# alibaba/unified-audio

Hardware: AMD Instinct MI355X
Metric: audio-seconds/sec H-Codec encode+decode @16kHz b=32 (higher is better)
Workload: dtype f32

## Files before the change

unified_audio_amd/csrc/conv_gemm.hip:

```cpp
#include <algorithm>
#include <cstdlib>
#include <type_traits>

#include "common.h"
#include "split_planes.h"

#ifndef QA_LOAD_AT
#define QA_LOAD_AT 0
#endif

#ifdef QA_TIMING
__device__ unsigned long long g_qa_timing[10];
extern "C" int qa_debug_timing(unsigned long long* out, int reset) {
    if (out && hipMemcpyFromSymbol(out, HIP_SYMBOL(g_qa_timing), sizeof(g_qa_timing)) != hipSuccess) return -1;
    if (reset) {
        unsigned long long z[10] = {0};
        if (hipMemcpyToSymbol(HIP_SYMBOL(g_qa_timing), z, sizeof(z)) != hipSuccess) return -1;
    }
    return 0;
}
#endif

namespace qa {

// ... 392 lines not shown
                    p.am_idx[m * p.am_ld + (ep_n >> 5)] = bi;
                }
                continue;
            }
            if (m >= p.M || ep_n >= p.N) continue;
            f32x4 v = *reinterpret_cast<const f32x4*>(stage + r * EP_LD + 4 * ep_c4);
            if (p.vec_epi) {
                v = epilogue4(v, p, m, ep_n, bias4, gamma4);
                *reinterpret_cast<f32x4*>(p.y + m * p.ldy + ep_n) = v;
            } else {
                for (int e = 0; e < 4 && ep_n + e < p.N; ++e) {
                    const int n = ep_n + e;
                    float u = v[e] + (p.bias ? p.bias[n] : 0.f);
                    if (p.gate) u = silu_f(p.gate[m * p.ldg + n]) * u;
                    u = apply_act(u, p.act);
                    if (p.gamma) u *= p.gamma[n];
                    if (p.res) u += p.res[m * p.ldr + n];
                    u = apply_act(u, p.post_act);
                    p.y[m * p.ldy + n] = u;
                }
            }
        }
    });
#ifdef QA_TIMING
    if (lane == 0) {
        const long long tend = __builtin_readcyclecounter();
        atomicAdd(&g_qa_timing[4], (unsigned long long)(tend - tloop));
        atomicAdd(&g_qa_timing[5], (unsigned long long)(tend - tbegin));
        atomicAdd(&g_qa_timing[6], 1ULL);
        atomicAdd(&g_qa_timing[7], (unsigned long long)nk);
        atomicAdd(&g_qa_timing[8], __builtin_amdgcn_s_memrealtime() - rbegin);
    }
#endif
}

static bool is_linear(const ConvParams& p) {
    return knob(K_GEMM_LINEAR) != 0 && p.ksize == 1 && p.stride == 1 && p.pad_left == 0 && p.in_rep <= 1 && p.T_in == p.T_out && p.dilation <= 1;
}

constexpr int prof_cfg(int bm, int bn) {
    return bm == 256 ? PROF_CFG_256x128 : bm == 64 ? (bn == 64 ? PROF_CFG_64x64 : PROF_CFG_64x128) : bn == 32 ? PROF_CFG_128x32 : bn == 64 ? PROF_CFG_128x64 : PROF_CFG_128x128;
}

template <int BM, int BN, int WM, int WN, bool ELU, int BK, bool LIN>
static void launch_instance(const ConvParams& p, long long tiles, hipStream_t stream) {
    const bool split = knob(K_GEMM_MATH) != 0 && !p.math_fp32;
    constexpr bool IMAGE = BN == 128;
    const auto kernel = !split            ? conv_gemm_kernel<BM, BN, WM, WN, ELU, BK, LIN, false, false>
                        : IMAGE && p.wp ? conv_gemm_kernel<BM, BN, WM, WN, ELU, BK, LIN, true, IMAGE>
                                        : conv_gemm_kernel<BM, BN, WM, WN, ELU, BK, LIN, true, false>;
    hipLaunchKernelGGL(kernel, dim3((unsigned)tiles), dim3(256), 0, stream, p);
}

template <int BM, int BN, int WM, int WN>
static int launch_cfg(const ConvParams& p, hipStream_t stream) {
    QA_REQUIRE(p.prologue == ACT_NONE || p.prologue == ACT_ELU, "conv_gemm: prologue %d unsupported", p.prologue);
    const long long tiles = ceil_div(p.M, BM) * ceil_div(p.N, BN);
    const long long bk16_max_k = knob(K_GEMM_BK16);
    const long long bk16_min_tiles = knob(K_GEMM_BK16_MIN_TILES);
    const bool linear = is_linear(p), elu = p.prologue == ACT_ELU;
    const bool bk16 = BM == 256 || (BN >= 64 && !elu && ((p.K <= bk16_max_k && tiles >= bk16_min_tiles) || p.C_in % 32 != 0));
    const int bk = bk16 ? 16 : 32;
    const bool table = BM != 256 && (!linear || elu);
    QA_REQUIRE(p.K % bk == 0 && (!table || p.C_in % bk == 0),
               "conv_gemm: the %dx%d tile's BK = %d K chunk does not divide K=%d / C_in=%d", BM, BN, bk, p.K, p.C_in);
    const bool prof = profile_enabled();
    if (prof) {
        const double n = p.algo_n ? p.algo_n : p.N, k = p.algo_k ? p.algo_k : p.K;
        const double out_elems = p.am_dist ? 2.0 * (double)p.M * p.am_ld + p.M + n
                                            : (double)p.M * n * (1.0 + (p.res ? 1.0 : 0.0) + (p.gate ? 1.0 : 0.0));
        const double elems = (double)p.B * p.T_in * p.C_in + n * k + out_elems;
        profile_record_begin(prof_cfg(BM, BN), 2.0 * (double)p.M * n * k, 4.0 * elems, stream, &p);
    }
    if constexpr (BM == 256) QA_REQUIRE(linear && !elu, "conv_gemm: the 256 x 128 tile exists for LINEAR layers only");
    constexpr int BK16 = BN >= 64 ? 16 : 32;
    if (bk16 && linear) launch_instance<BM, BN, WM, WN, false, BK16, true>(p, tiles, stream);
    else if constexpr (BM != 256) {
        if (bk16) launch_instance<BM, BN, WM, WN, false, BK16, false>(p, tiles, stream);
        else if (elu) launch_instance<BM, BN, WM, WN, true, 32, false>(p, tiles, stream);
        else if (linear) launch_instance<BM, BN, WM, WN, false, 32, true>(p, tiles, stream);
        else launch_instance<BM, BN, WM, WN, false, 32, false>(p, tiles, stream);
    }
    if (prof) profile_record_end(stream);
    QA_LAUNCH_CHECK();
    return QA_OK;
}

static int choose_tile(const ConvParams& p) {
    const bool lin = is_linear(p) && p.prologue != ACT_ELU;
    int cfg = (int)knob(K_GEMM_CFG);
    if (cfg < 0) {
        if (p.N <= 32) cfg = PROF_CFG_128x32;
        else if (p.N <= 64) cfg = PROF_CFG_128x64;
        else {
            struct Cand { int cfg, bm, bn; double eff; };
            static const Cand cands[] = {{PROF_CFG_128x128, 128, 128, 1.0}, {PROF_CFG_64x128, 64, 128, 0.914}, {PROF_CFG_128x64, 128, 64, 0.913},
                                         {PROF_CFG_64x64, 64, 64, 0.871}};
            auto cost_of = [&](int bm, int bn, double eff) {
                const long long tiles = ceil_div(p.M, bm) * ceil_div(p.N, bn);
                return (double)ceil_div(tiles, 256) * bm * bn / eff * (tiles <= 256 ? 1.25 : 1.0);
            };
            double best = 0.0;
            cfg = PROF_CFG_128x128;
            const long long eff256 = knob(K_GEMM_256);
            if (eff256 > 0 && lin && p.M >= 8000 && p.N >= 1024) {
                best = cost_of(256, 128, eff256 / 1000.0);
                cfg = PROF_CFG_256x128;
            }
            for (const Cand& c : cands) {
                const double cost = cost_of(c.bm, c.bn, c.eff);
                if (best == 0.0 || cost < best * 0.995) {
                    best = cost;
                    cfg = c.cfg;
                }
            }
        }
    }
    if (cfg == PROF_CFG_128x32 && p.C_in % 32 != 0) return PROF_CFG_128x64;
    if ((cfg == PROF_CFG_256x128 && !lin) || cfg >= PROF_NCFG) return PROF_CFG_128x128;
    return cfg;
}

int launch_conv_gemm(const ConvParams& p, hipStream_t stream) {
    QA_REQUIRE(p.K % 16 == 0 && p.C_in % 16 == 0, "conv_gemm: K=%d / C_in=%d must be multiples of 16", p.K, p.C_in);
    QA_REQUIRE(p.C_in % 32 == 0 || (p.N > 32 && p.prologue != ACT_ELU),
               "conv_gemm: C_in=%d is not a multiple of 32 (only supported for N > 32 without the ELU prologue)", p.C_in);
    QA_REQUIRE((p.ldx % 4) == 0, "conv_gemm: ldx=%lld must be a multiple of 4 floats", p.ldx);
    QA_REQUIRE((long long)p.T_in * p.ldx < (1LL << 31), "conv_gemm: one batch item spans %lld floats (limit 2^31)",
               (long long)p.T_in * p.ldx);
    QA_REQUIRE(((uintptr_t)p.x % 16) == 0 && ((uintptr_t)p.w % 16) == 0, "conv_gemm: x / w must be 16-byte aligned");
    if (p.M <= 0 || p.N <= 0) return QA_OK;
    QA_REQUIRE(ceil_div(p.M, 64) * ceil_div(p.N, 32) < (1LL << 31), "conv_gemm: grid too large");
    auto al16 = [](const void* ptr) { return ((uintptr_t)ptr % 16) == 0; };
    const bool vec_epi = p.N % 4 == 0 && p.ldy % 4 == 0 && al16(p.y) && (!p.bias || al16(p.bias)) && (!p.gamma || al16(p.gamma)) &&
                         (!p.res || (p.ldr % 4 == 0 && al16(p.res))) && (!p.gate || (p.ldg % 4 == 0 && al16(p.gate)));
    QA_REQUIRE(p.in_rep <= 1 || p.pad_mode == PAD_ZERO, "conv_gemm: in_rep needs zero padding");
    const bool snake = p.act == ACT_SNAKE || p.post_act == ACT_SNAKE;
    QA_REQUIRE((!snake && !p.y2) || (vec_epi && (!snake || (p.alpha && al16(p.alpha))) &&
                                     (!p.y2 || (p.alpha2 && al16(p.alpha2) && al16(p.y2) && p.ldy2 % 4 == 0))),
               "conv_gemm: Snake activation / second output need the float4 epilogue and 16-byte aligned alpha vectors");
    QA_REQUIRE(p.dilation <= 1 || (p.pad_mode == PAD_ZERO && p.in_rep <= 1), "conv_gemm: dilation needs zero padding");
    QA_REQUIRE(!p.am_dist || (vec_epi && p.am_idx && p.am_x2 && p.am_e2 && al16(p.am_e2) && p.am_ld >= (p.N + 31) / 32 && !p.y2),
               "conv_gemm: the arg-min epilogue needs N %% 4 == 0, x2 / e2 / dist / idx and am_ld >= ceil(N / 32)");
    QA_REQUIRE(!p.rope || (vec_epi && p.rope_hd % 4 == 0 && p.rope_n % 4 == 0 && p.rope_T > 0 && al16(p.rope)),
               "conv_gemm: fused RoPE needs the float4 epilogue (N, strides, pointers multiples of 4 / 16 B)");
    ConvParams q = p;
    q.xcd_swizzle = (int)knob(K_GEMM_XCD);
    q.panel = (int)knob(K_GEMM_PANEL);
    q.wp = knob(K_GEMM_PRESPLIT) != 0 ? weight_planes_find(p.w, (long long)p.N * p.K) : nullptr;
    q.vec_epi = vec_epi;
    q.rep_one = p.in_rep > 1 ? 0u : 1u;
    q.rep_magic = p.in_rep > 1 ? (unsigned)(((1ULL << 32) + p.in_rep - 1) / p.in_rep) : 0u;

    switch (choose_tile(p)) {
        case PROF_CFG_128x32: return launch_cfg<128, 32, 4, 1>(q, stream);
        case PROF_CFG_128x64: return launch_cfg<128, 64, 2, 2>(q, stream);
        case PROF_CFG_64x128: return launch_cfg<64, 128, 1, 4>(q, stream);
        case PROF_CFG_64x64: return launch_cfg<64, 64, 2, 2>(q, stream);
        case PROF_CFG_256x128: return launch_cfg<256, 128, 2, 2>(q, stream);
        default: return launch_cfg<128, 128, 2, 2>(q, stream);
    }
}

int conv_params_from_args(const qa_conv_args& a, ConvParams* out) {
    ConvParams p{};
    QA_REQUIRE(a.x && a.w && a.y, "conv1d_cl: x, w, y must be non-null");
    QA_REQUIRE(a.B > 0 && a.T_in > 0 && a.C_in > 0 && a.N > 0 && a.T_out >= 0, "conv1d_cl: bad shape");
    QA_REQUIRE(a.ksize >= 1 && a.stride >= 1 && a.pad_left >= 0 && a.pad_right >= 0, "conv1d_cl: bad geometry");
    QA_REQUIRE(a.B * a.T_out < (1LL << 31) && a.ksize * a.C_in < (1LL << 31), "conv1d_cl: shape too large");
    p.x = a.x; p.w = a.w; p.bias = a.bias; p.gamma = a.gamma; p.res = a.residual; p.gate = a.gate; p.y = a.y;
    p.ldx = a.ldx ? a.ldx : a.C_in;
    p.ldy = a.ldy ? a.ldy : a.N;
    p.ldr = a.ldr ? a.ldr : a.N;
    p.ldg = a.ldg ? a.ldg : a.N;
    p.B = (int)a.B; p.T_in = (int)a.T_in; p.C_in = (int)a.C_in; p.T_out = (int)a.T_out; p.N = (int)a.N;
    p.K = (int)(a.ksize * a.C_in);
    p.M = (int)(a.B * a.T_out);
    p.ksize = a.ksize; p.stride = a.stride; p.pad_left = a.pad_left; p.pad_mode = a.pad_mode;
    const int max_pad = a.pad_left > a.pad_right ? a.pad_left : a.pad_right;
    p.Lp = (p.T_in <= max_pad) ? max_pad + 1 : p.T_in;
    p.in_rep = a.in_rep > 1 ? a.in_rep : 1;
    QA_REQUIRE(a.T_out == 0 || (a.T_out - 1) * (int64_t)a.stride + a.ksize <= a.pad_left + a.T_in * (int64_t)p.in_rep + a.pad_right,
               "conv1d_cl: T_out=%lld windows do not fit pad_left=%d + T_in=%lld + pad_right=%d", (long long)a.T_out,
               a.pad_left, (long long)a.T_in, a.pad_right);
    p.prologue = a.prologue; p.act = a.act; p.post_act = a.post_act;
    *out = p;
    return QA_OK;
}

}
```

unified_audio_amd/csrc/ew.hip:

```cpp
#include "kernels.h"

namespace qa {

__global__ __launch_bounds__(256) void conv_in_kernel(const float* __restrict__ x, const float* __restrict__ w,
                                                      const float* __restrict__ bias, float* __restrict__ y, int B,
                                                      int T, int Cout, int ksize, int pad_left, int Lp) {
    const int c4n = Cout >> 2;
    const long long gid = (long long)blockIdx.x * blockDim.x + threadIdx.x;
    const long long total = (long long)B * T * c4n;
    if (gid >= total) return;
    const int c4 = (int)(gid % c4n);
    const long long m = gid / c4n;
    const int b = (int)(m / T), t = (int)(m - (long long)b * T);
    const float* xb = x + (long long)b * T;
    float4 acc = bias ? *reinterpret_cast<const float4*>(bias + c4 * 4) : make_float4(0.f, 0.f, 0.f, 0.f);
    for (int j = 0; j < ksize; ++j) {
        const int src = resolve_frame(t - pad_left + j, T, Lp, PAD_REFLECT);
        const float xv = src >= 0 ? xb[src] : 0.f;
        const float* wj = w + (long long)j * Cout + c4 * 4;
        acc.x = fmaf(xv, wj[0], acc.x);
        acc.y = fmaf(xv, wj[1], acc.y);
        acc.z = fmaf(xv, wj[2], acc.z);
        acc.w = fmaf(xv, wj[3], acc.w);
    }
// ... 510 lines not shown
    if (p < T) {
        const int dst = p + seg[(long long)b * T + p];
        for (int c = threadIdx.x * 4; c < D; c += blockDim.x * 4)
            *reinterpret_cast<float4*>(ob + (long long)dst * D + c) =
                *reinterpret_cast<const float4*>(feats + ((long long)b * T + p) * D + c);
        return;
    }
    const int g = p - T;
    if (g >= nseg[b]) {
        for (int c = threadIdx.x * 4; c < D; c += blockDim.x * 4)
            *reinterpret_cast<float4*>(ob + (long long)(T + g) * D + c) = *reinterpret_cast<const float4*>(qemb + c);
        return;
    }
    const int st = start[(long long)b * T + g], n = len[(long long)b * T + g];
    const int dst = st + n + g;
    const float inv = 1.f / (float)n;
    for (int c = threadIdx.x * 4; c < D; c += blockDim.x * 4) {
        float4 acc = make_float4(0.f, 0.f, 0.f, 0.f);
        for (int t = st; t < st + n; ++t) {
            const float4 v = *reinterpret_cast<const float4*>(feats + ((long long)b * T + t) * D + c);
            acc.x += v.x; acc.y += v.y; acc.z += v.z; acc.w += v.w;
        }
        const float4 q = *reinterpret_cast<const float4*>(qemb + c);
        acc.x = acc.x * inv + q.x; acc.y = acc.y * inv + q.y; acc.z = acc.z * inv + q.z; acc.w = acc.w * inv + q.w;
        *reinterpret_cast<float4*>(ob + (long long)dst * D + c) = acc;
    }
}
int launch_agg_build(const float* feats, const int* seg, const int* start, const int* len, const int* nseg, const float* qemb,
                     float* out, int B, int T, int G, int D, hipStream_t s) {
    hipLaunchKernelGGL(agg_build_kernel, dim3(T + G, B), dim3(128), 0, s, feats, seg, start, len, nseg, qemb, out, T, G, D);
    QA_LAUNCH_CHECK();
    return QA_OK;
}

__global__ __launch_bounds__(128) void agg_gather_kernel(const float* __restrict__ x, const int* __restrict__ start,
                                                         const int* __restrict__ len, const int* __restrict__ nseg,
                                                         float* __restrict__ out, int T, int G, int D) {
    const int b = blockIdx.y, g = blockIdx.x;
    const bool valid = g < nseg[b];
    const int src = valid ? start[(long long)b * T + g] + len[(long long)b * T + g] + g : 0;
    for (int c = threadIdx.x * 4; c < D; c += blockDim.x * 4) {
        float4 v = make_float4(0.f, 0.f, 0.f, 0.f);
        if (valid) v = *reinterpret_cast<const float4*>(x + ((long long)b * (T + G) + src) * D + c);
        *reinterpret_cast<float4*>(out + ((long long)b * G + g) * D + c) = v;
    }
}
int launch_agg_gather(const float* x, const int* start, const int* len, const int* nseg, float* out, int B, int T, int G,
                      int D, hipStream_t s) {
    hipLaunchKernelGGL(agg_gather_kernel, dim3(G, B), dim3(128), 0, s, x, start, len, nseg, out, T, G, D);
    QA_LAUNCH_CHECK();
    return QA_OK;
}

__global__ void codes_inject_kernel(const long long* __restrict__ idx, const int* __restrict__ len, long long* __restrict__ dst,
                                    int B, int T, int G, int Q, int K) {
    const long long gid = (long long)blockIdx.x * blockDim.x + threadIdx.x;
    if (gid >= (long long)B * Q * G) return;
    const int g = (int)(gid % G);
    const int q = (int)((gid / G) % Q);
    const int b = (int)(gid / ((long long)G * Q));
    dst[gid] = (long long)(len[(long long)b * T + g] - 1) * K + idx[((long long)b * G + g) * Q + q];
}
int launch_codes_inject(const long long* idx, const int* len, long long* dst, int B, int T, int G, int Q, int K,
                        hipStream_t s) {
    const long long total = (long long)B * Q * G;
    hipLaunchKernelGGL(codes_inject_kernel, dim3((unsigned)ceil_div(total, 256)), dim3(256), 0, s, idx, len, dst, B, T, G, Q, K);
    QA_LAUNCH_CHECK();
    return QA_OK;
}

__device__ __forceinline__ long long floordiv_ll(long long a, long long b) {
    long long q = a / b;
    if ((a % b != 0) && ((a < 0) != (b < 0))) --q;
    return q;
}

__global__ void adaptive_frames_kernel(const long long* __restrict__ codes, int B, int Q, int G, int K, int* __restrict__ totals,
                                       int* __restrict__ tmax) {
    const int b = blockIdx.x * blockDim.x + threadIdx.x;
    if (b >= B) return;
    int tot = 0;
    for (int g = 0; g < G; ++g) {
        const long long l = floordiv_ll(codes[((long long)b * Q) * G + g], K) + 1;
        tot += l > 0 ? (int)l : 0;
    }
    totals[b] = tot;
    atomicMax(tmax, tot);
}
int launch_adaptive_frames(const long long* codes, int B, int Q, int G, int K, int* totals, int* tmax, hipStream_t s) {
    QA_HIP(hipMemsetAsync(tmax, 0, sizeof(int), s));
    hipLaunchKernelGGL(adaptive_frames_kernel, dim3((unsigned)ceil_div(B, 64)), dim3(64), 0, s, codes, B, Q, G, K, totals, tmax);
    QA_LAUNCH_CHECK();
    return QA_OK;
}

__global__ void token_lengths_kernel(const long long* __restrict__ codes, long long* __restrict__ out, int B, int Q, int G, int K) {
    const long long gid = (long long)blockIdx.x * blockDim.x + threadIdx.x;
    if (gid >= (long long)B * G) return;
    const int g = (int)(gid % G), b = (int)(gid / G);
    out[gid] = floordiv_ll(codes[((long long)b * Q) * G + g], K) + 1;
}
int launch_token_lengths(const long long* codes, long long* out, int B, int Q, int G, int K, hipStream_t s) {
    const long long total = (long long)B * G;
    if (total == 0) return QA_OK;
    hipLaunchKernelGGL(token_lengths_kernel, dim3((unsigned)ceil_div(total, 256)), dim3(256), 0, s, codes, out, B, Q, G, K);
    QA_LAUNCH_CHECK();
// ... 125 lines not shown
```

unified_audio_amd/csrc/hcodec.cpp:

```cpp
#include <memory>

#include "host_util.h"

namespace qa {

namespace {

struct TransformerLayerW {
    const float *ln1, *ln2;
    ConvW ih;
    const float* w_hh;
    ConvW qkv, o, w1, w3, w2;
};

struct TransformerW {
    std::vector<TransformerLayerW> layers;
    int d = 0, heads = 0, inter = 0;
    const float* rope = nullptr;
};

struct ResBlockW {
    ConvW k3, pw, sc;
};
struct DecResW {
// ... 271 lines not shown
        QA_TRY(linear_op(c, hn, rows, L.w3, big2, epi(ACT_NONE, nullptr, nullptr, big)));
        QA_TRY(linear_op(c, big2, rows, L.w2, x, epi(ACT_NONE, x)));
        c.tap(lp + ".x_mlp", x, rows * d);
    }
    c.arena.release(mark);
    return QA_OK;
}

struct MimiTemps {
    float *hn, *qkv, *att, *u;
};
MimiTemps mimi_temps(Ctx& c, const MimiW& mw, int64_t rows) {
    MimiTemps t;
    t.hn = c.arena.alloc<float>(rows * mw.d);
    t.qkv = c.arena.alloc<float>(rows * 3 * mw.d);
    t.att = c.arena.alloc<float>(rows * mw.d);
    t.u = c.arena.alloc<float>(rows * mw.ff);
    return t;
}
int mimi_layer(Ctx& c, const MimiW& mw, const MimiLayerW& L, float* x, const MimiTemps& t, int B, int N, MimiStream* st = nullptr,
               size_t li = 0) {
    const int d = mw.d, H = mw.heads, hd = d / H;
    const int64_t rows = (int64_t)B * N;
    const int pos0 = st ? st->offset : 0;
    const bool win = st && st->rope_len > 0;
    const float* rope = win ? st->rope_win : mw.rope;
    const int rope_pos0 = win ? pos0 - st->rope_base : pos0;
    const float scale = 1.0f / std::sqrt((float)hd);
    QA_TRY(layernorm_op(c, x, L.n1w, L.n1b, t.hn, rows, d, 1e-5f));
    ConvOpt qo;
    qo.rope = rope; qo.rope_n = 2 * d; qo.rope_hd = hd; qo.rope_T = N; qo.rope_pos0 = rope_pos0;
    QA_TRY(linear_op(c, t.hn, rows, L.in_proj, t.qkv, qo));
    if (st) {
        QA_RUN(c, launch_ring_append(t.qkv + d, t.qkv + 2 * d, 3 * d, st->kc[li], st->vc[li], B, N, d, st->cap, pos0, c.stream));
        QA_TRY(attention_op(c, t.qkv, 3 * d, st->kc[li], st->vc[li], d, t.att, d, B, N, st->cap, (long long)st->cap * d, H, hd, scale, 1,
                            nullptr, nullptr, 0, mw.context, pos0, pos0 + N));
    } else {
        QA_TRY(attention_op(c, t.qkv, 3 * d, t.qkv + d, t.qkv + 2 * d, 3 * d, t.att, d, B, N, N, (long long)N * 3 * d, H, hd, scale,
                            mw.causal, nullptr, nullptr, 0, mw.causal ? mw.context : 0));
    }
    QA_TRY(linear_op(c, t.att, rows, L.out_proj, x, epi(ACT_NONE, x, L.ls1)));
    QA_TRY(layernorm_op(c, x, L.n2w, L.n2b, t.hn, rows, d, 1e-5f));
    QA_TRY(linear_op(c, t.hn, rows, L.lin1, t.u, epi(ACT_GELU)));
    return linear_op(c, t.u, rows, L.lin2, x, epi(ACT_NONE, x, L.ls2));
}
int mimi_op(Ctx& c, const MimiW& mw, float* x, int B, int N) {
    QA_REQUIRE(N <= MAX_POS, "mimi transformer: sequence of %d tokens exceeds %d", N, MAX_POS);
    const size_t mark = c.arena.mark();
    const MimiTemps t = mimi_temps(c, mw, (int64_t)B * N);
    for (const MimiLayerW& L : mw.layers) QA_TRY(mimi_layer(c, mw, L, x, t, B, N));
    c.arena.release(mark);
    return QA_OK;
}
int mimi_pair_op(Ctx& c, hipStream_t side, const MimiW& wa, float* xa, const MimiW& wb, float* xb, int B, int N) {
    QA_REQUIRE(N <= MAX_POS && wa.layers.size() == wb.layers.size(), "mimi pair: mismatched stacks");
    const size_t mark = c.arena.mark();
    const MimiTemps ta = mimi_temps(c, wa, (int64_t)B * N);
    const MimiTemps tb = mimi_temps(c, wb, (int64_t)B * N);
    if (!c.dry) {
        hipStream_t main = c.stream;
        for (size_t l = 0; l < wa.layers.size(); ++l) {
            c.stream = main;
            int st = mimi_layer(c, wa, wa.layers[l], xa, ta, B, N);
            c.stream = side;
            if (st == QA_OK) st = mimi_layer(c, wb, wb.layers[l], xb, tb, B, N);
            c.stream = main;
            QA_TRY(st);
        }
    }
    c.arena.release(mark);
    return QA_OK;
}

int groupnorm_op(Ctx& c, const float* x, const float* w, const float* b, float* y, int B, int T, int C, int G,
                 int swish) {
    const size_t mark = c.arena.mark();
    double* scratch = c.arena.alloc<double>(groupnorm_scratch_bytes(B, T, G) / sizeof(double));
    QA_RUN(c, launch_groupnorm(x, w, b, y, scratch, B, T, C, G, 1e-6f, swish, c.stream));
    c.arena.release(mark);
    return QA_OK;
}

int dec_resblock_op(Ctx& c, const DecResW& w, float* x, int B, int T, int C, int G, bool causal = false) {
    const size_t mark = c.arena.mark();
    float* t1 = c.arena.alloc<float>((size_t)B * T * C);
    float* t2 = c.arena.alloc<float>((size_t)B * T * C);
    QA_TRY(groupnorm_op(c, x, w.n1w, w.n1b, t1, B, T, C, G, 1));
    QA_TRY(conv_same(c, t1, B, T, w.c1, t2, ACT_NONE, ACT_NONE, nullptr, causal));
    QA_TRY(groupnorm_op(c, t2, w.n2w, w.n2b, t1, B, T, C, G, 1));
    QA_TRY(conv_same(c, t1, B, T, w.c2, x, ACT_NONE, ACT_NONE, x, causal));
    c.arena.release(mark);
    return QA_OK;
}


int convnext_op(Ctx& c, const ConvNeXtW& w, float* x, float* t1, float* u, int B, int T, int d, bool causal = false) {
    const int64_t rows = (int64_t)B * T;
    QA_TRY(dwconv_op(c, x, w.dw, w.dwb, w.lnw, w.lnb, t1, B, T, d, 7, 1e-6f, zpad_left(7, causal)));
    QA_TRY(linear_op(c, t1, rows, w.pw1, u, epi(ACT_GELU)));
    return linear_op(c, u, rows, w.pw2, x, epi(ACT_NONE, x, w.gamma));
}

int encoder20(qa_hcodec* h, Ctx& c, const float* wav, int B, int T, float** emb_out, int* n50_out, int* nf_out) {
    const qa_hcodec_spec& sp = h->spec;
    const int blk = (sp.n_fft - sp.hop) / 2;
    const int N50 = T / sp.hop, d = sp.enc_dim, nb = sp.n_fft / 2 + 1;
    const int64_t rows = (int64_t)B * N50;
    float* ri = c.arena.alloc<float>(rows * 2 * nb);
    QA_TRY(conv_op(c, wav, blk, B, T / blk, h->stft_basis, ri, 2 * nb, N50, conv_geom(2, 1, 1)));
    float* feat = c.arena.alloc<float>(rows * h->stft_ld);
    QA_RUN(c, launch_stft_post(ri, feat, rows, nb, 2 * nb, h->stft_ld, c.stream));
    c.tap("enc.stft", feat, rows * h->stft_ld);
    float* x = c.arena.alloc<float>(rows * d);
    float* t1 = c.arena.alloc<float>(rows * d);
    float* u = c.arena.alloc<float>(rows * sp.enc_inter);
    const bool cz = sp.causal != 0;
    QA_TRY(conv_op(c, feat, h->stft_ld, B, N50, h->enc_embed, t1, d, N50, conv_geom(1, cz ? 2 : 1, cz ? 0 : 1)));
    QA_TRY(layernorm_op(c, t1, h->enc_norm_w, h->enc_norm_b, x, rows, d, 1e-6f));
// ... 179 lines not shown
    c.tap("dec.backbone", t1, rows * d);
    const int nb = sp.n_fft / 2 + 1;
    float* y = c.arena.alloc<float>(rows * 2 * nb);
    float* S = c.arena.alloc<float>(rows * h->spec_ld);
    float* frames = c.arena.alloc<float>(rows * sp.n_fft);
    QA_TRY(linear_op(c, t1, rows, h->head, y));
    QA_RUN(c, launch_istft_spec(y, S, rows, nb, 2 * nb, h->spec_ld, c.stream));
    c.tap("dec.spec", S, rows * h->spec_ld);
    QA_TRY(linear_op(c, S, rows, h->basis, frames));
    QA_RUN(c, launch_istft_ola(frames, h->window, wav_out, B, N50, sp.n_fft, sp.hop, c.stream));
    return QA_OK;
}


int read_scalar(Ctx& c, qa_hcodec* h, const int* dev, int* out) {
    QA_HIP(hipMemcpyAsync(h->host_sync, dev, sizeof(int), hipMemcpyDeviceToHost, c.stream));
    QA_HIP(hipStreamSynchronize(c.stream));
    lstm_call_note_sync();
    *out = *h->host_sync;
    return QA_OK;
}

int encode_adaptive_graph(qa_hcodec* h, Ctx& c, const float* wav, int B, int T, const float* feat, int64_t fsb, int64_t fsc,
                          int64_t fst, int n_feat, long long* ac_out, long long* sc_out, int* G_out, float threshold) {
    const qa_hcodec_spec& sp = h->spec;
    const int D = sp.code_dim, Q = sp.num_quantizers;
    float *emb = nullptr, *sem = nullptr;
    int N = 0;
    QA_TRY(encode_front(h, c, wav, B, T, feat, fsb, fsc, fst, n_feat, &emb, &sem, &N));
    int* seg = c.arena.alloc<int>((size_t)B * N);
    int* start = c.arena.alloc<int>((size_t)B * N);
    int* len = c.arena.alloc<int>((size_t)B * N);
    int* nseg = c.arena.alloc<int>(B);
    int* gmax = c.arena.alloc<int>(1);
    int G = N;
    if (!c.dry) {
        QA_TRY(launch_align(sem, B, N, D, threshold, sp.max_tokens_per_group, seg, start, len, nseg, gmax, c.stream));
        QA_TRY(read_scalar(c, h, gmax, &G));
        QA_REQUIRE(G >= 1 && G <= N, "encode: alignment produced %d groups for %d frames", G, N);
    }
    *G_out = G;
    const int S = N + G;
    float* inter_s = c.arena.alloc<float>((size_t)B * S * D);
    float* inter_a = c.arena.alloc<float>((size_t)B * S * D);
    float* agg_a = c.arena.alloc<float>((size_t)B * G * D);
    float* agg_s = c.arena.alloc<float>((size_t)B * G * D);
    hipStream_t side = serial_mode() ? c.stream : h->side;
    QA_RUN(c, launch_agg_build(sem, seg, start, len, nseg, h->qemb_sem, inter_s, B, N, G, D, c.stream));
    QA_RUN(c, launch_agg_build(emb, seg, start, len, nseg, h->qemb_ac, inter_a, B, N, G, D, c.stream));
    if (!c.dry) {
        QA_HIP(hipEventRecord(h->ev_fork, c.stream));
        QA_HIP(hipStreamWaitEvent(side, h->ev_fork, 0));
    }
    QA_TRY(mimi_pair_op(c, side, h->agg_sem, inter_s, h->agg_ac, inter_a, B, S));
    QA_RUN(c, launch_agg_gather(inter_s, start, len, nseg, agg_s, B, N, G, D, c.stream));
    QA_RUN(c, launch_agg_gather(inter_a, start, len, nseg, agg_a, B, N, G, D, side));
    if (!c.dry) {
        QA_HIP(hipEventRecord(h->ev_join, side));
        QA_HIP(hipStreamWaitEvent(c.stream, h->ev_join, 0));
    }
    c.tap("enc.emb_agg", agg_a, (int64_t)B * G * D);
    c.tap("enc.sem_agg", agg_s, (int64_t)B * G * D);
    long long* ia = c.arena.alloc<long long>((size_t)B * G * Q);
    long long* is = c.arena.alloc<long long>((size_t)B * G * Q);
    float* rvq_ws = c.arena.alloc<float>(rvq_scratch_floats((long long)B * G, sp.codebook_size, D));
    QA_RUN(c, launch_rvq_search(agg_a, (long long)B * G, h->cb_a, h->e2_a, Q, sp.codebook_size, D, ia, nullptr, 0, rvq_ws, c.stream));
    QA_RUN(c, launch_rvq_search(agg_s, (long long)B * G, h->cb_s, h->e2_s, Q, sp.codebook_size, D, is, nullptr, 0, rvq_ws, c.stream));
    QA_RUN(c, launch_codes_inject(ia, len, ac_out, B, N, G, Q, sp.codebook_size, c.stream));
    QA_RUN(c, launch_codes_inject(is, len, sc_out, B, N, G, Q, sp.codebook_size, c.stream));
    return QA_OK;
}

int decode_adaptive_graph(qa_hcodec* h, Ctx& c, const long long* ac, const long long* scodes, int B, int G, int N,
                          float* wav_out) {
    const qa_hcodec_spec& sp = h->spec;
    const int Q = sp.num_quantizers, D = sp.code_dim;
    const int64_t rows = (int64_t)B * N;
    long long* ia = c.arena.alloc<long long>(rows * Q);
    long long* is = c.arena.alloc<long long>(rows * Q);
    float* cat = c.arena.alloc<float>(rows * 2 * D);
    QA_RUN(c, launch_deaggregate(ac, scodes, ia, B, Q, G, N, sp.codebook_size, c.stream));
    QA_RUN(c, launch_deaggregate(scodes, scodes, is, B, Q, G, N, sp.codebook_size, c.stream));
    QA_RUN(c, launch_rvq_lookup(ia, rows, h->cb_a, Q, sp.codebook_size, D, cat, 2 * D, c.stream));
    QA_RUN(c, launch_rvq_lookup(is, rows, h->cb_s, Q, sp.codebook_size, D, cat + D, 2 * D, c.stream));
    QA_TRY(mimi_op(c, h->bottleneck, cat, B, N));
    c.tap("dec.bottleneck", cat, rows * 2 * D);
    return decode_tail(h, c, cat, B, N, wav_out);
}


int semantic_decoder_op(const qa_hcodec::SemDec& sd, Ctx& c, const float* z, int64_t ldz, int B, int N, float* pred) {
    const qa_semantic_decoder_spec& sp = sd.spec;
    int L = N, C = sp.channels;
    float* x = c.arena.alloc<float>((size_t)B * L * C);
    QA_TRY(conv_op(c, z, ldz, B, L, sd.conv1, x, C, L, conv_geom(1, 1, 1)));
    for (const auto& blk : sd.blocks) {
        const int s = blk.stride, co = blk.c_out, To = L * s;
        float* y = c.arena.alloc<float>((size_t)B * To * co);
        if (s == 1) {
            QA_TRY(conv_same(c, x, B, L, blk.conv, y));
        } else {
            for (int phi = 0; phi < s; ++phi) {
                const ConvW& w = blk.phase[phi];
                QA_TRY(conv_op(c, x, C, B, L, w, y + (size_t)phi * co, (int64_t)s * co, L,
                               conv_geom(1, blk.pad_left[phi], w.ksize - 1 - blk.pad_left[phi])));
            }
        }
        float* t = c.arena.alloc<float>((size_t)B * To * co);
        for (int u = 0; u < 2; ++u) {
// ... 666 lines not shown
```

unified_audio_amd/csrc/kernels.h:

```cpp
#pragma once
#include <algorithm>

#include "common.h"

namespace qa {

int launch_conv_in(const float* x, const float* w_kc, const float* bias, float* y, int B, int T, int Cout, int ksize,
                   hipStream_t s, int pad_left = -1);
bool seanet_front_supported(int C, int hid, int L);
int launch_seanet_front(const float* wav, const float* w0, const float* b0, const float* w3, const float* b3, const float* wsc,
                        const float* bsc, const float* wpw, const float* bpw, float* a, int B, int L, int C, int hid, int causal,
                        hipStream_t s);
int launch_rmsnorm(const float* x, const float* w, float* y, long long rows, int C, float eps, hipStream_t s);
int launch_layernorm(const float* x, const float* w, const float* b, float* y, long long rows, int C, float eps,
                     hipStream_t s);
int launch_dwconv(const float* x, const float* w_kc, const float* bias, const float* lnw, const float* lnb, float* y,
                  int B, int T, int C, int ksize, float eps, hipStream_t s, int pad_left = -1);
size_t groupnorm_scratch_bytes(int B, int T, int G);
int launch_groupnorm(const float* x, const float* w, const float* bias, float* y, double* scratch, int B, int T, int C,
                     int G, float eps, int swish, hipStream_t s);
int launch_rope(float* qkv, const float* cos_sin, int B, int N, int H, int hd, long long ld, int pos0, hipStream_t s,
                int interleaved = 0, int rot_heads = 0);
int launch_align(const float* sem, int B, int T, int D, float thr, int max_tokens, int* seg, int* start, int* len,
                 int* nseg, int* gmax, hipStream_t s);
int launch_agg_build(const float* feats, const int* seg, const int* start, const int* len, const int* nseg, const float* qemb,
                     float* out, int B, int T, int G, int D, hipStream_t s);
int launch_agg_gather(const float* x, const int* start, const int* len, const int* nseg, float* out, int B, int T, int G,
                      int D, hipStream_t s);
int launch_codes_inject(const long long* idx, const int* len, long long* dst, int B, int T, int G, int Q, int K,
                        hipStream_t s);
int launch_adaptive_frames(const long long* codes, int B, int Q, int G, int K, int* totals, int* tmax, hipStream_t s);
int launch_token_lengths(const long long* codes, long long* out, int B, int Q, int G, int K, hipStream_t s);
int launch_deaggregate(const long long* codes, const long long* len_codes, long long* out, int B, int Q, int G, int T, int K,
                       hipStream_t s);
int launch_to_channel_last(const float* x, long long sb, long long sc, long long st, float* y, int B, int C, int T,
                           hipStream_t s);
int launch_codes_to_bqn(const long long* src, long long* dst, int B, int N, int Q, hipStream_t s);
int launch_codes_from_bqn(const long long* src, long long* dst, int B, int N, int Q, hipStream_t s);
int launch_stft_post(const float* ri, float* out, long long rows, int nb, int ldi, int ldo, hipStream_t s);
int launch_istft_spec(const float* y, float* S, long long rows, int nb, int ldy, int ldS, hipStream_t s);
int launch_istft_ola(const float* frames, const float* win, float* out, int B, int T, int n_fft, int hop, hipStream_t s);

int launch_codes_check(const long long* codes, long long n, long long limit, unsigned long long* bad, hipStream_t s);
int launch_codes_count(const long long* codes, long long n, long long lo, long long limit, unsigned long long* bad, hipStream_t s);
int launch_resample(const float* wav, const float* taps, float* out, int B, long long T, long long T_out, int orig, int nw, int width,
                    int ktaps, hipStream_t s);

int launch_attention(const float* q, long long ldq, const float* k, const float* v, long long ldkv, float* out,
                     long long ldo, int B, int n_q, int n_keys, long long kv_batch_stride, int H, int hd, float scale,
                     int causal, hipStream_t s, const float* gate = nullptr, const float* relbias = nullptr, int R = 0,
                     int context = 0, int q_pos0 = 0, int ring_end = 0, const unsigned char* kvalid = nullptr, bool math_fp32 = false);
int launch_ring_append(const float* k, const float* v, long long ld, float* kc, float* vc, int B, int T, int d, int cap, int pos0,
                       hipStream_t s);

int launch_lstm(const float* xw, const float* w_hh_ug, float* h_out, float* c_state, int B, int T, int d,
                hipStream_t s, bool eager = false);
int lstm_call_begin(int dev, void** ticket);
int lstm_call_end(void* ticket, hipStream_t s, bool* failed);
void lstm_call_note_sync();
void lstm_force_per_step(bool on);

size_t rvq_scratch_floats(long long n_vec, int K, int D);
int launch_rvq_search(const float* x, long long n_vec, const float* codebooks, const float* e2, int Q, int K, int D,
                      long long* indices, float* quantized, long long ldq, float* scratch, hipStream_t s);
int launch_rvq_norms(const float* codebooks, float* e2, int QK, int D, hipStream_t s);
int launch_rvq_lookup(const long long* indices, long long n_vec, const float* codebooks, int Q, int K, int D, float* out,
                      long long ldo, hipStream_t s);

int launch_assemble_prompt(float* x, const float* task_vec, const float* enroll_sos, const float* enroll_emb,
                           const float* mix_sos, const float* mix_emb, int B, int Ne, int Nm, int d, hipStream_t s,
                           const int* off = nullptr);
int launch_skinny_gemm(const float* x, long long ldx, const float* w, const float* bias, const float* gate, long long ldg,
                       const float* res, long long ldr, float* y, long long ldy, int M, int N, int K, int act, hipStream_t s,
                       float rms_eps, int dual);
int launch_rope_kv(float* qkv, const float* cs, float* kc, float* vc, int B, int n, int H, int hd, int pos0, int max_len,
                   hipStream_t s);
int launch_lm_targets(float* x, long long ldx_seq, const float* table, const long long* gids, int G, const long long* sids, int T, int V,
                      int goff, int soff, long long* tgt, int B, int d, hipStream_t s, int drop = 0);
int launch_lm_row_loss(const float* z, long long ldl, int V, long long rows, const long long* tgt, float c, float sm, float* row_kl,
                       int* row_ok, hipStream_t s);
int launch_lm_seq_reduce(const float* row_kl, const int* row_ok, int B, int Lt, double* seq_sum, float* loss_seq, long long* correct_seq,
// ... 53 lines not shown
```

unified_audio_amd/csrc/knobs.h:

```cpp
#pragma once
#include <cstdint>

namespace qa {

#define QA_KNOB_TABLE(X)                                                                                                           \
    X(SERIAL, "QA_SERIAL", 0, "1: no internal stream concurrency (every kernel alone on the device; = qa_set_serial)")           \
    X(GEMM_CFG, "QA_GEMM_CFG", -1, "force the conv_gemm tile: 0 = 128x32, 1 = 128x64, 2 = 128x128, 3 = 64x128, 4 = 64x64, 5 = 256x128 (LINEAR layers; else 128x128) (-1: cost model)")             \
    X(GEMM_256, "QA_GEMM_256", 0, "r06 experiment: 256x128 block tile (4 waves, 4x2 accumulators each) for LINEAR layers with M >= 8000 and N >= 1024; value = its efficiency relative to 128x128 in 1/1000 for the cost model (0: never chosen; QA_GEMM_CFG=5 forces it)") \
    X(GEMM_BK16, "QA_GEMM_BK16", 1 << 30, "largest K that takes the BK = 16 K-chunk variant")                                     \
    X(GEMM_BK16_MIN_TILES, "QA_GEMM_BK16_MIN_TILES", 384, "fewest tiles of a launch that take BK = 16")                          \
    X(GEMM_MATH, "QA_GEMM_MATH", 1, "conv_gemm arithmetic: 1 = split-6 (operands split into three bf16 planes, six v_mfma_f32_32x32x16_bf16 per 16-wide k group, fp32 accumulation), 0 = the fp32 chain (v_mfma_f32_32x32x2_f32)") \
    X(GEMM_PRESPLIT, "QA_GEMM_PRESPLIT", 1, "split-6 weights from a pre-split image: a weight store builds the three bf16 planes of all its weights once, at load (6 bytes per weight beside the fp32 blob; not built when 0 at load time), and conv_gemm's 128-column tiles copy them into LDS instead of splitting the weight tile in the K loop (narrower tiles keep the in-loop split); 0 at launch = ignore the image and split in the loop; same bits either way") \
    X(GEMM_LINEAR, "QA_GEMM_LINEAR", 1, "table-free K loop for ksize-1 layers")                                                  \
    X(GEMM_XCD, "QA_GEMM_XCD", 1, "XCD-aware tile order")                                                                        \
    X(GEMM_PANEL, "QA_GEMM_PANEL", 8, "conv_gemm tile order: column panels of this many tiles, row tiles fastest inside a panel (0: column tiles fastest over the whole row; 8: +4 % on N >= 4096 shapes, +1.2 % on H-Codec 2.0)") \
    X(ATT_MATH, "QA_ATT_MATH", 1, "attention arithmetic: 1 = split-6 (Q, K, V and the probabilities as three bf16 planes, six v_mfma_f32_32x32x16_bf16 per 16-wide k group, fp32 accumulation), 0 = the fp32 chain (v_mfma_f32_32x32x2_f32); the UniSE LM keeps the fp32 chain either way") \
    X(ATT_DEBUG, "QA_ATT_DEBUG", 0, "attention_kernel debug bits, both forms: 1 always rescale, 2 extra barrier per tile, 4 wait for the prefetch at once, 8 no wave-uniform tile skip, 16 mask every tile; the split-6 form (SPLIT) only (tests): 32 / 64 / 128 zero the h / m / l plane of the operands selected by 256 Q, 512 K, 1024 V, 2048 P (none of the four: all)") \
    X(SEANET_FUSED, "QA_SEANET_FUSED", 1, "fused conv0 + first SEANet residual block")                                           \
    X(MIMI_ROPE_WINDOW, "QA_MIMI_ROPE_WINDOW", 8192, "mimi streaming: positions covered by the RoPE table before the rolling window takes over (tests shrink it)") \
    X(LSTM_GRAPH, "QA_LSTM_GRAPH", 1, "replay the T step launches of an LSTM call from a cached hipGraph")                       \
    X(LSTM_PERSISTENT, "QA_LSTM_PERSISTENT", -1, "persistent recurrence kernel: -1 auto (d >= 1536), 0 off, 1 on for every supported width") \
    X(LSTM_XCD, "QA_LSTM_XCD", 1, "XCD-local LSTM recurrence for d = 512 / 768 (one launch, W_hh in the registers of every XCD's 32 CUs, sequences dealt to the XCDs, 32-member step barrier per XCD): 0 off (the per-step kernels), 1 agent-scope hand-off forms, 2 XCD-local forms (h stores that stay in the XCD's L2; H-Codec 1.0: 42.7 against 43.3 ms)") \
    X(LSTM_TEAM, "QA_LSTM_TEAM", 1, "team recurrence for d = 1024 (one launch: 4 teams of 64 workgroups, W_hh resident in registers, 8 sequences per team, agent-scope hand-offs; H-Codec 1.5 decoder: 134.1 -> 128.3 ms per step, profiles/r04_lstm_team_ab.txt): 0 = the per-step kernels") \
    X(LSTM_SPIN_LIMIT, "QA_LSTM_SPIN_LIMIT", 1 << 21, "persistent recurrence: polls of a barrier word before the barrier is declared broken") \
    X(LSTM_FAULT, "QA_LSTM_FAULT", 0, "1 (tests): the persistent kernel's barrier waits for a workgroup that does not exist, like a starved launch") \
    X(LM_GRAPH, "QA_LM_GRAPH", 0, "1: replay one captured decode step per token")                                                \
    X(LM_MLP_FUSED, "QA_LM_MLP_FUSED", 1, "decode step: gate/up + SwiGLU + down of 16 activation columns per workgroup in one launch emitting K-slice partials, summed by a reduce launch (0: separate gate/up and down launches)") \
    X(LM_PF, "QA_LM_PF", 7, "decode step: cross-launch L2 weight prefetch planes (bit mask; lm_decode.h PfArgs): 1 qkv launch -> o_proj weights, 2 o_proj launch -> fused-MLP weights, 4 MLP launch -> next layer's qkv weights (last layer: the head slice), 8 head launch -> layer 0 qkv weights") \
    X(LM_ROWSPLIT, "QA_LM_ROWSPLIT", 3, "decode step at 9 .. 16 sequences: two 8-row groups instead of one 16-row group in the qkv launch (bit 1) and the fused-MLP launch (bit 2)") \
    X(LM_CHAINS, "QA_LM_CHAINS", 0, "generate: number of concurrent chains on internal streams (0: ceil(B / 64) - one chain serves up to 64 sequences, two row groups of 32 per launch; a count that would put more than 64 sequences into a chain is raised)") \
    X(LM_SCORE_ROWS, "QA_LM_SCORE_ROWS", 4096, "qa_lm_score: target rows per output_head launch (the logits buffer holds this many rows of the full vocabulary; any value gives the same bits)")

enum Knob {
#define QA_KNOB_ENUM(id, name, def, doc) K_##id,
    QA_KNOB_TABLE(QA_KNOB_ENUM)
#undef QA_KNOB_ENUM
        K_COUNT
};

long long knob(Knob k);
void knob_set(Knob k, long long v);

}
```

Before: 3139.

## Compute only read-out rows in last aggregator layer; occupancy-aware GEMM tile cost

Result: faster. 3272, median of 6 (+4.2%).

```diff
diff --git a/unified_audio_amd/csrc/conv_gemm.hip b/unified_audio_amd/csrc/conv_gemm.hip
--- a/unified_audio_amd/csrc/conv_gemm.hip
+++ b/unified_audio_amd/csrc/conv_gemm.hip
@@ -468,14 +468,16 @@
     hipLaunchKernelGGL(kernel, dim3((unsigned)tiles), dim3(256), 0, stream, p);
 }
 
+static bool takes_bk16(int bm, int bn, long long tiles, int K, int C_in, bool elu) {
+    return bm == 256 || (bn >= 64 && !elu && ((K <= knob(K_GEMM_BK16) && tiles >= knob(K_GEMM_BK16_MIN_TILES)) || C_in % 32 != 0));
+}
+
 template <int BM, int BN, int WM, int WN>
 static int launch_cfg(const ConvParams& p, hipStream_t stream) {
     QA_REQUIRE(p.prologue == ACT_NONE || p.prologue == ACT_ELU, "conv_gemm: prologue %d unsupported", p.prologue);
     const long long tiles = ceil_div(p.M, BM) * ceil_div(p.N, BN);
-    const long long bk16_max_k = knob(K_GEMM_BK16);
-    const long long bk16_min_tiles = knob(K_GEMM_BK16_MIN_TILES);
     const bool linear = is_linear(p), elu = p.prologue == ACT_ELU;
-    const bool bk16 = BM == 256 || (BN >= 64 && !elu && ((p.K <= bk16_max_k && tiles >= bk16_min_tiles) || p.C_in % 32 != 0));
+    const bool bk16 = takes_bk16(BM, BN, tiles, p.K, p.C_in, elu);
     const int bk = bk16 ? 16 : 32;
     const bool table = BM != 256 && (!linear || elu);
     QA_REQUIRE(p.K % bk == 0 && (!table || p.C_in % bk == 0),
@@ -502,29 +504,56 @@
     return QA_OK;
 }
 
-static int choose_tile(const ConvParams& p) {
-    const bool lin = is_linear(p) && p.prologue != ACT_ELU;
+struct TileQuery {
+    long long M, N, K;
+    int C_in;
+    bool lin, elu, split;
+    bool image;
+    int share;
+};
+static int workgroups_per_cu(int cfg, bool bk16, bool split) {
+    switch (cfg) {
+        case PROF_CFG_128x128: return bk16 ? 3 : split ? 1 : 2;
+        case PROF_CFG_64x128: return bk16 ? 4 : 2;
+        case PROF_CFG_128x64: return bk16 ? 4 : 2;
+        case PROF_CFG_64x64: return bk16 ? 5 : split ? 3 : 4;
+        case PROF_CFG_256x128: return 2;
+        default: return split ? 2 : 3;
+    }
+}
+static double tile_cost(const TileQuery& t, int cfg, int bm, int bn, double eff) {
+    constexpr double kTile = 128.0 * 128.0, kRamp = 0.22, kLaunch = 0.27 * 512.0;
+    const long long tiles = ceil_div(t.M, bm) * ceil_div(t.N, bn);
+    const long long w = workgroups_per_cu(cfg, takes_bk16(bm, bn, tiles, (int)t.K, t.C_in, t.elu), t.split);
+    const long long n = tiles * (t.share > 1 ? t.share : 1), cap = 256 * w;
+    const long long rounds = ceil_div(n, cap), m = n - (rounds - 1) * cap;
+    double last = 0.5 * ((double)ceil_div(m, 256) + (double)m / 256.0);
+    if (last < 1.0) last = 1.0;
+    return kTile * kLaunch + (double)t.K * ((double)bm * bn / eff * ((double)(w * (rounds - 1)) + last) + kRamp * kTile * (double)rounds);
+}
+static double tile_cost_r4(const TileQuery& t, int bm, int bn, double eff) {
+    const long long tiles = ceil_div(t.M, bm) * ceil_div(t.N, bn);
+    return (double)ceil_div(tiles, 256) * bm * bn / eff * (tiles <= 256 ? 1.25 : 1.0);
+}
+static int choose_tile(const TileQuery& t) {
     int cfg = (int)knob(K_GEMM_CFG);
     if (cfg < 0) {
-        if (p.N <= 32) cfg = PROF_CFG_128x32;
-        else if (p.N <= 64) cfg = PROF_CFG_128x64;
+        if (t.N <= 32) cfg = PROF_CFG_128x32;
+        else if (t.N <= 64) cfg = PROF_CFG_128x64;
         else {
-            struct Cand { int cfg, bm, bn; double eff; };
-            static const Cand cands[] = {{PROF_CFG_128x128, 128, 128, 1.0}, {PROF_CFG_64x128, 64, 128, 0.914}, {PROF_CFG_128x64, 128, 64, 0.913},
-                                         {PROF_CFG_64x64, 64, 64, 0.871}};
-            auto cost_of = [&](int bm, int bn, double eff) {
-                const long long tiles = ceil_div(p.M, bm) * ceil_div(p.N, bn);
-                return (double)ceil_div(tiles, 256) * bm * bn / eff * (tiles <= 256 ? 1.25 : 1.0);
-            };
+            struct Cand { int cfg, bm, bn; double eff6, eff32; };
+            static const Cand cands[] = {{PROF_CFG_128x128, 128, 128, 1.0, 1.0}, {PROF_CFG_64x128, 64, 128, 0.85, 0.914},
+                                         {PROF_CFG_128x64, 128, 64, 0.80, 0.913}, {PROF_CFG_64x64, 64, 64, 0.69, 0.871}};
             double best = 0.0;
             cfg = PROF_CFG_128x128;
             const long long eff256 = knob(K_GEMM_256);
-            if (eff256 > 0 && lin && p.M >= 8000 && p.N >= 1024) {
-                best = cost_of(256, 128, eff256 / 1000.0);
+            const bool r4 = t.split && !t.image;
+            if (eff256 > 0 && t.lin && t.M >= 8000 && t.N >= 1024) {
+                best = r4 ? tile_cost_r4(t, 256, 128, eff256 / 1000.0) : tile_cost(t, PROF_CFG_256x128, 256, 128, eff256 / 1000.0);
                 cfg = PROF_CFG_256x128;
             }
             for (const Cand& c : cands) {
-                const double cost = cost_of(c.bm, c.bn, c.eff);
+                const double cost = r4 ? tile_cost_r4(t, c.bm, c.bn, c.eff32) : tile_cost(t, c.cfg, c.bm, c.bn, t.split ? c.eff6 : c.eff32);
                 if (best == 0.0 || cost < best * 0.995) {
                     best = cost;
                     cfg = c.cfg;
@@ -532,9 +561,13 @@
             }
         }
     }
-    if (cfg == PROF_CFG_128x32 && p.C_in % 32 != 0) return PROF_CFG_128x64;
-    if ((cfg == PROF_CFG_256x128 && !lin) || cfg >= PROF_NCFG) return PROF_CFG_128x128;
+    if (cfg == PROF_CFG_128x32 && t.C_in % 32 != 0) return PROF_CFG_128x64;
+    if ((cfg == PROF_CFG_256x128 && !t.lin) || cfg >= PROF_NCFG) return PROF_CFG_128x128;
     return cfg;
+}
+static int choose_tile(const ConvParams& p) {
+    const bool elu = p.prologue == ACT_ELU;
+    return choose_tile(TileQuery{p.M, p.N, p.K, p.C_in, is_linear(p) && !elu, elu, knob(K_GEMM_MATH) != 0 && !p.math_fp32, p.wp != nullptr, 1});
 }
 
 int launch_conv_gemm(const ConvParams& p, hipStream_t stream) {
@@ -568,7 +601,7 @@
     q.rep_one = p.in_rep > 1 ? 0u : 1u;
     q.rep_magic = p.in_rep > 1 ? (unsigned)(((1ULL << 32) + p.in_rep - 1) / p.in_rep) : 0u;
 
-    switch (choose_tile(p)) {
+    switch (choose_tile(q)) {
         case PROF_CFG_128x32: return launch_cfg<128, 32, 4, 1>(q, stream);
         case PROF_CFG_128x64: return launch_cfg<128, 64, 2, 2>(q, stream);
         case PROF_CFG_64x128: return launch_cfg<64, 128, 1, 4>(q, stream);
@@ -605,3 +638,12 @@
 }
 
 }
+
+extern "C" int qa_debug_conv_gemm_tile(long long M, long long N, long long K, int ksize, int linear, int math_fp32, int share) {
+    if (M <= 0 || N <= 0 || K <= 0 || ksize < 1 || K % ksize != 0 || M >= (1LL << 31) || N >= (1LL << 31) || K >= (1LL << 31)) {
+        qa::set_error("qa_debug_conv_gemm_tile: bad argument");
+        return -1;
+    }
+    const bool lin = linear != 0 && ksize == 1 && qa::knob(qa::K_GEMM_LINEAR) != 0;
+    return qa::choose_tile(qa::TileQuery{M, N, K, (int)(K / ksize), lin, false, qa::knob(qa::K_GEMM_MATH) != 0 && !math_fp32, true, share});
+}
diff --git a/unified_audio_amd/csrc/ew.hip b/unified_audio_amd/csrc/ew.hip
--- a/unified_audio_amd/csrc/ew.hip
+++ b/unified_audio_amd/csrc/ew.hip
@@ -586,6 +586,37 @@
     return QA_OK;
 }
 
+__global__ __launch_bounds__(128) void agg_query_rows_kernel(const float* __restrict__ x, const float* __restrict__ qkv,
+                                                             const int* __restrict__ start, const int* __restrict__ len,
+                                                             const int* __restrict__ nseg, float* __restrict__ xq,
+                                                             float* __restrict__ qq, int T, int G, int D) {
+    const int b = blockIdx.y, g = blockIdx.x;
+    const int src = g < nseg[b] ? start[(long long)b * T + g] + len[(long long)b * T + g] + g : 0;
+    const long long row = (long long)b * (T + G) + src, dst = ((long long)b * G + g) * D;
+    for (int c = threadIdx.x * 4; c < D; c += blockDim.x * 4) {
+        *reinterpret_cast<float4*>(xq + dst + c) = *reinterpret_cast<const float4*>(x + row * D + c);
+        *reinterpret_cast<float4*>(qq + dst + c) = *reinterpret_cast<const float4*>(qkv + row * 3 * D + c);
+    }
+}
+int launch_agg_query_rows(const float* x, const float* qkv, const int* start, const int* len, const int* nseg, float* xq, float* qq,
+                          int B, int T, int G, int D, hipStream_t s) {
+    QA_REQUIRE(D % 4 == 0, "agg_query_rows: D=%d must be a multiple of 4", D);
+    hipLaunchKernelGGL(agg_query_rows_kernel, dim3(G, B), dim3(128), 0, s, x, qkv, start, len, nseg, xq, qq, T, G, D);
+    QA_LAUNCH_CHECK();
+    return QA_OK;
+}
+__global__ __launch_bounds__(128) void agg_zero_padded_kernel(const int* __restrict__ nseg, float* __restrict__ out, int G, int D) {
+    const int b = blockIdx.y, g = blockIdx.x;
+    if (g < nseg[b]) return;
+    for (int c = threadIdx.x * 4; c < D; c += blockDim.x * 4)
+        *reinterpret_cast<float4*>(out + ((long long)b * G + g) * D + c) = make_float4(0.f, 0.f, 0.f, 0.f);
+}
+int launch_agg_zero_padded(const int* nseg, float* out, int B, int G, int D, hipStream_t s) {
+    hipLaunchKernelGGL(agg_zero_padded_kernel, dim3(G, B), dim3(128), 0, s, nseg, out, G, D);
+    QA_LAUNCH_CHECK();
+    return QA_OK;
+}
+
 __global__ void codes_inject_kernel(const long long* __restrict__ idx, const int* __restrict__ len, long long* __restrict__ dst,
                                     int B, int T, int G, int Q, int K) {
     const long long gid = (long long)blockIdx.x * blockDim.x + threadIdx.x;
diff --git a/unified_audio_amd/csrc/hcodec.cpp b/unified_audio_amd/csrc/hcodec.cpp
--- a/unified_audio_amd/csrc/hcodec.cpp
+++ b/unified_audio_amd/csrc/hcodec.cpp
@@ -347,18 +347,48 @@
     c.arena.release(mark);
     return QA_OK;
 }
-int mimi_pair_op(Ctx& c, hipStream_t side, const MimiW& wa, float* xa, const MimiW& wb, float* xb, int B, int N) {
+struct AggReadout {
+    const int *start, *len, *nseg;
+    int T, G;
+    float* out;
+};
+int mimi_readout_layer(Ctx& c, const MimiW& mw, const MimiLayerW& L, const float* x, const MimiTemps& t, float* xq, float* qq, int B,
+                       const AggReadout& ro) {
+    const int d = mw.d, H = mw.heads, hd = d / H, N = ro.T + ro.G;
+    const int64_t rows = (int64_t)B * N, qrows = (int64_t)B * ro.G;
+    QA_TRY(layernorm_op(c, x, L.n1w, L.n1b, t.hn, rows, d, 1e-5f));
+    ConvOpt qo;
+    qo.rope = mw.rope; qo.rope_n = 2 * d; qo.rope_hd = hd; qo.rope_T = N; qo.rope_pos0 = 0;
+    QA_TRY(linear_op(c, t.hn, rows, L.in_proj, t.qkv, qo));
+    QA_RUN(c, launch_agg_query_rows(x, t.qkv, ro.start, ro.len, ro.nseg, xq, qq, B, ro.T, ro.G, d, c.stream));
+    QA_TRY(attention_op(c, qq, d, t.qkv + d, t.qkv + 2 * d, 3 * d, t.att, d, B, ro.G, N, (long long)N * 3 * d, H, hd,
+                        1.0f / std::sqrt((float)hd), 0));
+    QA_TRY(linear_op(c, t.att, qrows, L.out_proj, xq, epi(ACT_NONE, xq, L.ls1)));
+    QA_TRY(layernorm_op(c, xq, L.n2w, L.n2b, t.hn, qrows, d, 1e-5f));
+    QA_TRY(linear_op(c, t.hn, qrows, L.lin1, t.u, epi(ACT_GELU)));
+    QA_TRY(linear_op(c, t.u, qrows, L.lin2, ro.out, epi(ACT_NONE, xq, L.ls2)));
+    QA_RUN(c, launch_agg_zero_padded(ro.nseg, ro.out, B, ro.G, d, c.stream));
+    return QA_OK;
+}
+int mimi_pair_op(Ctx& c, hipStream_t side, const MimiW& wa, float* xa, const MimiW& wb, float* xb, int B, int N,
+                 const AggReadout* ra = nullptr, const AggReadout* rb = nullptr) {
     QA_REQUIRE(N <= MAX_POS && wa.layers.size() == wb.layers.size(), "mimi pair: mismatched stacks");
+    QA_REQUIRE(!ra == !rb && (!ra || (!wa.causal && !wb.causal && wa.d == wb.d && !wa.layers.empty())), "mimi pair: bad read-out");
     const size_t mark = c.arena.mark();
     const MimiTemps ta = mimi_temps(c, wa, (int64_t)B * N);
     const MimiTemps tb = mimi_temps(c, wb, (int64_t)B * N);
+    float* cq[4] = {nullptr, nullptr, nullptr, nullptr};
+    if (ra)
+        for (float*& p : cq) p = c.arena.alloc<float>((size_t)B * ra->G * wa.d);
     if (!c.dry) {
         hipStream_t main = c.stream;
         for (size_t l = 0; l < wa.layers.size(); ++l) {
+            const bool last = ra && l + 1 == wa.layers.size();
             c.stream = main;
-            int st = mimi_layer(c, wa, wa.layers[l], xa, ta, B, N);
+            int st = last ? mimi_readout_layer(c, wa, wa.layers[l], xa, ta, cq[0], cq[1], B, *ra) : mimi_layer(c, wa, wa.layers[l], xa, ta, B, N);
             c.stream = side;
-            if (st == QA_OK) st = mimi_layer(c, wb, wb.layers[l], xb, tb, B, N);
+            if (st == QA_OK)
+                st = last ? mimi_readout_layer(c, wb, wb.layers[l], xb, tb, cq[2], cq[3], B, *rb) : mimi_layer(c, wb, wb.layers[l], xb, tb, B, N);
             c.stream = main;
             QA_TRY(st);
         }
@@ -644,9 +674,14 @@
         QA_HIP(hipEventRecord(h->ev_fork, c.stream));
         QA_HIP(hipStreamWaitEvent(side, h->ev_fork, 0));
     }
-    QA_TRY(mimi_pair_op(c, side, h->agg_sem, inter_s, h->agg_ac, inter_a, B, S));
-    QA_RUN(c, launch_agg_gather(inter_s, start, len, nseg, agg_s, B, N, G, D, c.stream));
-    QA_RUN(c, launch_agg_gather(inter_a, start, len, nseg, agg_a, B, N, G, D, side));
+    if (knob(K_AGG_LAST_ROWS) != 0 && !h->agg_sem.causal && !h->agg_ac.causal && !h->agg_sem.layers.empty()) {
+        const AggReadout rs{start, len, nseg, N, G, agg_s}, ra{start, len, nseg, N, G, agg_a};
+        QA_TRY(mimi_pair_op(c, side, h->agg_sem, inter_s, h->agg_ac, inter_a, B, S, &rs, &ra));
+    } else {
+        QA_TRY(mimi_pair_op(c, side, h->agg_sem, inter_s, h->agg_ac, inter_a, B, S));
+        QA_RUN(c, launch_agg_gather(inter_s, start, len, nseg, agg_s, B, N, G, D, c.stream));
+        QA_RUN(c, launch_agg_gather(inter_a, start, len, nseg, agg_a, B, N, G, D, side));
+    }
     if (!c.dry) {
         QA_HIP(hipEventRecord(h->ev_join, side));
         QA_HIP(hipStreamWaitEvent(c.stream, h->ev_join, 0));
diff --git a/unified_audio_amd/csrc/kernels.h b/unified_audio_amd/csrc/kernels.h
--- a/unified_audio_amd/csrc/kernels.h
+++ b/unified_audio_amd/csrc/kernels.h
@@ -27,6 +27,9 @@
                      float* out, int B, int T, int G, int D, hipStream_t s);
 int launch_agg_gather(const float* x, const int* start, const int* len, const int* nseg, float* out, int B, int T, int G,
                       int D, hipStream_t s);
+int launch_agg_query_rows(const float* x, const float* qkv, const int* start, const int* len, const int* nseg, float* xq, float* qq,
+                          int B, int T, int G, int D, hipStream_t s);
+int launch_agg_zero_padded(const int* nseg, float* out, int B, int G, int D, hipStream_t s);
 int launch_codes_inject(const long long* idx, const int* len, long long* dst, int B, int T, int G, int Q, int K,
                         hipStream_t s);
 int launch_adaptive_frames(const long long* codes, int B, int Q, int G, int K, int* totals, int* tmax, hipStream_t s);
diff --git a/unified_audio_amd/csrc/knobs.h b/unified_audio_amd/csrc/knobs.h
--- a/unified_audio_amd/csrc/knobs.h
+++ b/unified_audio_amd/csrc/knobs.h
@@ -16,6 +16,7 @@
     X(GEMM_PANEL, "QA_GEMM_PANEL", 8, "conv_gemm tile order: column panels of this many tiles, row tiles fastest inside a panel (0: column tiles fastest over the whole row; 8: +4 % on N >= 4096 shapes, +1.2 % on H-Codec 2.0)") \
     X(ATT_MATH, "QA_ATT_MATH", 1, "attention arithmetic: 1 = split-6 (Q, K, V and the probabilities as three bf16 planes, six v_mfma_f32_32x32x16_bf16 per 16-wide k group, fp32 accumulation), 0 = the fp32 chain (v_mfma_f32_32x32x2_f32); the UniSE LM keeps the fp32 chain either way") \
     X(ATT_DEBUG, "QA_ATT_DEBUG", 0, "attention_kernel debug bits, both forms: 1 always rescale, 2 extra barrier per tile, 4 wait for the prefetch at once, 8 no wave-uniform tile skip, 16 mask every tile; the split-6 form (SPLIT) only (tests): 32 / 64 / 128 zero the h / m / l plane of the operands selected by 256 Q, 512 K, 1024 V, 2048 P (none of the four: all)") \
+    X(AGG_LAST_ROWS, "QA_AGG_LAST_ROWS", 1, "H-Codec 1.5 encode: the last layer of each aggregator stack runs attention, out_proj, LayerNorm 2, lin1 and lin2 on the G query rows per clip only (the rows the read-out keeps); 0 = the full last layer; same bits either way") \
     X(SEANET_FUSED, "QA_SEANET_FUSED", 1, "fused conv0 + first SEANet residual block")                                           \
     X(MIMI_ROPE_WINDOW, "QA_MIMI_ROPE_WINDOW", 8192, "mimi streaming: positions covered by the RoPE table before the rolling window takes over (tests shrink it)") \
     X(LSTM_GRAPH, "QA_LSTM_GRAPH", 1, "replay the T step launches of an LSTM call from a cached hipGraph")                       \
```
